# DavidHan008/SLAM-1

Hardware: AMD Instinct MI355X
Metric: frames/sec tracking+local-BA @1280x720 (higher is better)
Workload: dtype u8+f32+f64

## Files before the change

slam-1_amd/csrc/epnp.hpp:

```cpp
#pragma once

#include <hip/hip_runtime.h>
#include <cmath>
#include <cstddef>

namespace slam_epnp {

constexpr int EPNP_MAXN = 8;
constexpr int kEpnpWs = 4 * EPNP_MAXN + 48 + 60;

template <int n>
__device__ __forceinline__ void ep_jacobi(double* A, double* V) {
  #pragma unroll
  for (int i = 0; i < n; ++i)
    #pragma unroll
    for (int j = 0; j < n; ++j) V[i * n + j] = i == j ? 1.0 : 0.0;
  #pragma unroll 1
  for (int sweep = 0; sweep < 40; ++sweep) {
    double off = 0.0, dia = 0.0;
    #pragma unroll
    for (int i = 0; i < n; ++i) {
      dia += A[i * n + i] * A[i * n + i];
      #pragma unroll
      for (int j = i + 1; j < n; ++j) off += A[i * n + j] * A[i * n + j];
    }
    if (!(off > 1e-30 * dia)) break;
    constexpr int kUnroll = n <= 4 ? 4 : 1;
    #pragma unroll kUnroll
    for (int p = 0; p < n - 1; ++p)
      #pragma unroll kUnroll
      for (int q = p + 1; q < n; ++q) {
        const double apq = A[p * n + q];
        if (apq == 0.0) continue;
        const double app = A[p * n + p], aqq = A[q * n + q];
        const double th = (aqq - app) / (2.0 * apq);
        const double t = (th >= 0.0 ? 1.0 : -1.0) / (fabs(th) + sqrt(th * th + 1.0));
        const double c = 1.0 / sqrt(t * t + 1.0), s = t * c;
        #pragma unroll
        for (int k = 0; k < n; ++k) {
          const double akp = A[k * n + p], akq = A[k * n + q];
          A[k * n + p] = c * akp - s * akq;
          A[k * n + q] = s * akp + c * akq;
        }
        #pragma unroll
        for (int k = 0; k < n; ++k) {
          const double apk = A[p * n + k], aqk = A[q * n + k];
          A[p * n + k] = c * apk - s * aqk;
          A[q * n + k] = s * apk + c * aqk;
        }
        #pragma unroll
        for (int k = 0; k < n; ++k) {
          const double vkp = V[k * n + p], vkq = V[k * n + q];
          V[k * n + p] = c * vkp - s * vkq;
          V[k * n + q] = s * vkp + c * vkq;
        }
      }
  }
}

template <int k>
__device__ __forceinline__ int ep_lsq6(const double* A, const double* b, double* x) {
  double N[5][5], r[5];
  #pragma unroll
  for (int i = 0; i < k; ++i) {
    #pragma unroll
    for (int j = 0; j <= i; ++j) {
      double s = 0.0;
      #pragma unroll
      for (int m = 0; m < 6; ++m) s += A[m * k + i] * A[m * k + j];
      N[i][j] = s;
    }
    double s = 0.0;
    #pragma unroll
    for (int m = 0; m < 6; ++m) s += A[m * k + i] * b[m];
    r[i] = s;
  }
  #pragma unroll
  for (int j = 0; j < k; ++j) {
    double s = N[j][j];
    #pragma unroll
    for (int p = 0; p < j; ++p) s -= N[j][p] * N[j][p];
    if (!(s > 0.0)) return 0;
    N[j][j] = sqrt(s);
    #pragma unroll
    for (int i = j + 1; i < k; ++i) {
      double t = N[i][j];
      #pragma unroll
      for (int p = 0; p < j; ++p) t -= N[i][p] * N[j][p];
      N[i][j] = t / N[j][j];
    }
  }
  double y[5];
  #pragma unroll
  for (int i = 0; i < k; ++i) {
    double t = r[i];
    #pragma unroll
    for (int p = 0; p < i; ++p) t -= N[i][p] * y[p];
    y[i] = t / N[i][i];
  }
  #pragma unroll
  for (int i = k - 1; i >= 0; --i) {
    double t = y[i];
    #pragma unroll
    for (int p = i + 1; p < k; ++p) t -= N[p][i] * x[p];
    x[i] = t / N[i][i];
  }
  return 1;
}

// ... 72 lines not shown
  double c0[3] = {0, 0, 0}, w0[3] = {0, 0, 0};
  #pragma unroll
  for (int i = 0; i < n; ++i)
    #pragma unroll
    for (int d = 0; d < 3; ++d) {
      c0[d] += pc[i][d];
      w0[d] += pw[3 * i + d];
    }
  #pragma unroll
  for (int d = 0; d < 3; ++d) {
    c0[d] /= n;
    w0[d] /= n;
  }
  double S[3][3] = {{0, 0, 0}, {0, 0, 0}, {0, 0, 0}};
  #pragma unroll
  for (int i = 0; i < n; ++i)
    #pragma unroll
    for (int a = 0; a < 3; ++a)
      #pragma unroll
      for (int b = 0; b < 3; ++b) S[a][b] += (pw[3 * i + a] - w0[a]) * (pc[i][b] - c0[b]);
  double N[16] = {S[0][0] + S[1][1] + S[2][2], S[1][2] - S[2][1], S[2][0] - S[0][2], S[0][1] - S[1][0],
                  S[1][2] - S[2][1], S[0][0] - S[1][1] - S[2][2], S[0][1] + S[1][0], S[2][0] + S[0][2],
                  S[2][0] - S[0][2], S[0][1] + S[1][0], -S[0][0] + S[1][1] - S[2][2], S[1][2] + S[2][1],
                  S[0][1] - S[1][0], S[2][0] + S[0][2], S[1][2] + S[2][1], -S[0][0] - S[1][1] + S[2][2]};
  double V[16];
  ep_jacobi<4>(N, V);
  int bi = 0;
  #pragma unroll
  for (int i = 1; i < 4; ++i)
    if (N[i * 4 + i] > N[bi * 4 + bi]) bi = i;
  double q0 = V[0 * 4 + bi], q1 = V[1 * 4 + bi], q2 = V[2 * 4 + bi], q3 = V[3 * 4 + bi];
  if (q0 < 0.0) {
    q0 = -q0; q1 = -q1; q2 = -q2; q3 = -q3;
  }
  R[0] = q0 * q0 + q1 * q1 - q2 * q2 - q3 * q3;
  R[1] = 2.0 * (q1 * q2 - q0 * q3);
  R[2] = 2.0 * (q1 * q3 + q0 * q2);
  R[3] = 2.0 * (q1 * q2 + q0 * q3);
  R[4] = q0 * q0 - q1 * q1 + q2 * q2 - q3 * q3;
  R[5] = 2.0 * (q2 * q3 - q0 * q1);
  R[6] = 2.0 * (q1 * q3 - q0 * q2);
  R[7] = 2.0 * (q2 * q3 + q0 * q1);
  R[8] = q0 * q0 - q1 * q1 - q2 * q2 + q3 * q3;
  #pragma unroll
  for (int d = 0; d < 3; ++d) t[d] = c0[d] - (R[3 * d] * w0[0] + R[3 * d + 1] * w0[1] + R[3 * d + 2] * w0[2]);
  double err = 0.0;
  #pragma unroll
  for (int i = 0; i < n; ++i) {
    const double* X = pw + 3 * i;
    const double Xc = R[0] * X[0] + R[1] * X[1] + R[2] * X[2] + t[0];
    const double Yc = R[3] * X[0] + R[4] * X[1] + R[5] * X[2] + t[1];
    const double Zc = R[6] * X[0] + R[7] * X[1] + R[8] * X[2] + t[2];
    const double du = cx + fx * Xc / Zc - uv[2 * i], dv = cy + fy * Yc / Zc - uv[2 * i + 1];
    err += sqrt(du * du + dv * dv);
  }
  return err / n;
}

__device__ inline void ep_rvec(const double R[9], double r[3]) {
  const double tr = R[0] + R[4] + R[8];
  double q0, q1, q2, q3;
  if (tr > 0.0) {
    const double s = 2.0 * sqrt(tr + 1.0);
    q0 = 0.25 * s; q1 = (R[7] - R[5]) / s; q2 = (R[2] - R[6]) / s; q3 = (R[3] - R[1]) / s;
  } else if (R[0] > R[4] && R[0] > R[8]) {
    const double s = 2.0 * sqrt(1.0 + R[0] - R[4] - R[8]);
    q0 = (R[7] - R[5]) / s; q1 = 0.25 * s; q2 = (R[1] + R[3]) / s; q3 = (R[2] + R[6]) / s;
  } else if (R[4] > R[8]) {
    const double s = 2.0 * sqrt(1.0 + R[4] - R[0] - R[8]);
    q0 = (R[2] - R[6]) / s; q1 = (R[1] + R[3]) / s; q2 = 0.25 * s; q3 = (R[5] + R[7]) / s;
  } else {
    const double s = 2.0 * sqrt(1.0 + R[8] - R[0] - R[4]);
    q0 = (R[3] - R[1]) / s; q1 = (R[2] + R[6]) / s; q2 = (R[5] + R[7]) / s; q3 = 0.25 * s;
  }
  if (q0 < 0.0) {
    q0 = -q0; q1 = -q1; q2 = -q2; q3 = -q3;
  }
  const double vn = sqrt(q1 * q1 + q2 * q2 + q3 * q3);
  const double th = 2.0 * atan2(vn, q0);
  const double k = vn > 0.0 ? th / vn : 2.0;
  r[0] = q1 * k; r[1] = q2 * k; r[2] = q3 * k;
}

constexpr int kJld = 13;
struct EpGroup {
  double A[144], V[144];
  double alph[4 * EPNP_MAXN];
  double cw[4][3];
  double offdia[2];
  double B[2][12 * kJld];
  double cs[12];
  double part[24];
  double pad[3];
  int o12[4];
  int flag;
};
static_assert(sizeof(EpGroup) % 256 == 128, "EpGroup stride must be 128 mod 256 bytes");

struct EpBeta {
  double flag;
  double pw[3 * 5], uv[2 * 5];
  double alph[4 * 5];
  double cw[4][3];
  double v[4][12];
  double L[60], rho[6];
  double res[3][8];
};
constexpr int kEpRec = 1 + 15 + 10 + 20 + 12 + 48;
static_assert(offsetof(EpBeta, L) == kEpRec * sizeof(double), "EpBeta starts with the record");
static_assert(sizeof(EpBeta) % 64 == 32, "EpBeta stride must be 4 mod 8 doubles");

template <int n>
__device__ __forceinline__ int ep_bary(const double* pw, EpGroup& G) {
  double cw[4][3] = {{0, 0, 0}};
  for (int i = 0; i < n; ++i)
    for (int d = 0; d < 3; ++d) cw[0][d] += pw[3 * i + d];
  for (int d = 0; d < 3; ++d) cw[0][d] /= n;
  double A3[9] = {0, 0, 0, 0, 0, 0, 0, 0, 0}, V3[9];
  for (int i = 0; i < n; ++i)
    for (int a = 0; a < 3; ++a)
      for (int b = 0; b < 3; ++b) A3[3 * a + b] += (pw[3 * i + a] - cw[0][a]) * (pw[3 * i + b] - cw[0][b]);
  ep_jacobi<3>(A3, V3);
  int ord[3] = {0, 1, 2};
  for (int i = 0; i < 3; ++i)
    for (int j = i + 1; j < 3; ++j)
      if (A3[4 * ord[j]] > A3[4 * ord[i]]) {
        const int tmp = ord[i]; ord[i] = ord[j]; ord[j] = tmp;
      }
  for (int k = 0; k < 3; ++k) {
    const double sc = sqrt(fmax(A3[4 * ord[k]], 0.0) / n);
    for (int d = 0; d < 3; ++d) cw[k + 1][d] = cw[0][d] + sc * V3[3 * d + ord[k]];
  }
  for (int k = 0; k < 4; ++k)
    for (int d = 0; d < 3; ++d) G.cw[k][d] = cw[k][d];
  double C[3][3];
  for (int d = 0; d < 3; ++d)
    for (int k = 0; k < 3; ++k) C[d][k] = cw[k + 1][d] - cw[0][d];
  const double c00 = C[1][1] * C[2][2] - C[1][2] * C[2][1];
  const double c01 = C[0][2] * C[2][1] - C[0][1] * C[2][2];
  const double c02 = C[0][1] * C[1][2] - C[0][2] * C[1][1];
  const double c10 = C[1][2] * C[2][0] - C[1][0] * C[2][2];
  const double c11 = C[0][0] * C[2][2] - C[0][2] * C[2][0];
  const double c12 = C[0][2] * C[1][0] - C[0][0] * C[1][2];
  const double c20 = C[1][0] * C[2][1] - C[1][1] * C[2][0];
  const double c21 = C[0][1] * C[2][0] - C[0][0] * C[2][1];
  const double c22 = C[0][0] * C[1][1] - C[0][1] * C[1][0];
  const double det = C[0][0] * c00 + C[0][1] * c10 + C[0][2] * c20;
  if (!(fabs(det) > 0.0)) return 0;
  const double id = 1.0 / det;
  for (int i = 0; i < n; ++i) {
    const double x = pw[3 * i] - cw[0][0], y = pw[3 * i + 1] - cw[0][1], z = pw[3 * i + 2] - cw[0][2];
    const double a1 = (c00 * x + c01 * y + c02 * z) * id;
    const double a2 = (c10 * x + c11 * y + c12 * z) * id;
    const double a3 = (c20 * x + c21 * y + c22 * z) * id;
    G.alph[4 * i] = 1.0 - a1 - a2 - a3;
    G.alph[4 * i + 1] = a1;
    G.alph[4 * i + 2] = a2;
    G.alph[4 * i + 3] = a3;
  }
  return 1;
}

template <int n>
__device__ __forceinline__ void ep_mtm_row(int r, const double* uv, double fx, double fy, double cx,
                                           double cy, EpGroup& G) {
  double acc[12];
#pragma unroll
  for (int c = 0; c < 12; ++c) acc[c] = 0.0;
  const int jr = r / 3, dr = r - 3 * jr;
  for (int i = 0; i < n; ++i) {
    double m1[12], m2[12];
#pragma unroll
    for (int j = 0; j < 4; ++j) {
      const double a = G.alph[4 * i + j];
      m1[3 * j] = a * fx; m1[3 * j + 1] = 0.0; m1[3 * j + 2] = a * (cx - uv[2 * i]);
      m2[3 * j] = 0.0; m2[3 * j + 1] = a * fy; m2[3 * j + 2] = a * (cy - uv[2 * i + 1]);
    }
    const double ar = G.alph[4 * i + jr];
    const double m1r = dr == 0 ? ar * fx : dr == 1 ? 0.0 : ar * (cx - uv[2 * i]);
    const double m2r = dr == 0 ? 0.0 : dr == 1 ? ar * fy : ar * (cy - uv[2 * i + 1]);
#pragma unroll
    for (int c = 0; c < 12; ++c) acc[c] += m1r * m1[c] + m2r * m2[c];
  }
#pragma unroll
  for (int c = 0; c < 12; ++c) G.A[12 * r + c] = acc[c];
}

__device__ __forceinline__ void ep_pairs12(int r, int pp[6], int qq[6]) {
  int a[12];
  a[0] = 0;
#pragma unroll
  for (int i = 1; i < 12; ++i) a[i] = 1 + (i - 1 + r) % 11;
#pragma unroll
  for (int i = 0; i < 6; ++i) {
    const int x = a[i], y = a[11 - i];
    pp[i] = x < y ? x : y;
    qq[i] = x < y ? y : x;
  }
}

__device__ __forceinline__ void ep_rot_cs(double app, double aqq, double apq, double& c, double& s) {
  const bool z = apq == 0.0;
  const double th = (aqq - app) / (2.0 * (z ? 1.0 : apq));
  const double t = (th >= 0.0 ? 1.0 : -1.0) / (fabs(th) + sqrt(th * th + 1.0));
  const double cc = 1.0 / sqrt(t * t + 1.0);
  c = z ? 1.0 : cc;
  s = z ? 0.0 : t * cc;
}

template <int r>
__device__ __forceinline__ void ep_jacobi_round(EpGroup& G, int k, int kr, bool act, int cur,
                                                double (&vr)[12]) {
  constexpr int n = 12, ld = kJld;
  const double* A0 = G.B[cur];
  double* A1 = G.B[cur ^ 1];
  int pp[6], qq[6];
  ep_pairs12(r, pp, qq);
  if (k < 6) {
    const int x = k == 0 ? 0 : 1 + (k - 1 + r) % 11, y = 1 + (10 - k + r) % 11;
    const int p = x < y ? x : y, q = x < y ? y : x;
    double c, s;
    ep_rot_cs(A0[p * ld + p], A0[q * ld + q], A0[p * ld + q], c, s);
    G.cs[2 * k] = c;
    G.cs[2 * k + 1] = s;
  }
  const int pos = kr == 0 ? 0 : (kr + 10 - r % 11) % 11 + 1;
  const int ppos = 11 - pos;
  const int partner = ppos == 0 ? 0 : 1 + (ppos - 1 + r) % 11;
  const int pi = pos < ppos ? pos : ppos;
  const bool isp = kr < partner;
  double row[n], prow[n];
#pragma unroll
  for (int j = 0; j < n; ++j) {
    row[j] = A0[kr * ld + j];
    prow[j] = A0[partner * ld + j];
  }
  __syncthreads();
  double c[6], s[6];
#pragma unroll
  for (int i = 0; i < 6; ++i) {
    c[i] = G.cs[2 * i];
    s[i] = G.cs[2 * i + 1];
  }
  double ck = c[0], sk = s[0];
#pragma unroll
  for (int i = 1; i < 6; ++i) {
    ck = pi == i ? c[i] : ck;
    sk = pi == i ? s[i] : sk;
  }
  double out[n];
#pragma unroll
  for (int j = 0; j < n; ++j) out[j] = row[j];
#pragma unroll
  for (int i = 0; i < 6; ++i) {
    const int P = pp[i], Q = qq[i];
    const double akp = row[P], akq = row[Q];
    row[P] = c[i] * akp - s[i] * akq;
    row[Q] = s[i] * akp + c[i] * akq;
    const double bkp = prow[P], bkq = prow[Q];
    prow[P] = c[i] * bkp - s[i] * bkq;
    prow[Q] = s[i] * bkp + c[i] * bkq;
    const double vkp = vr[P], vkq = vr[Q];
    const double wp = c[i] * vkp - s[i] * vkq, wq = s[i] * vkp + c[i] * vkq;
    vr[P] = act ? wp : vkp;
    vr[Q] = act ? wq : vkq;
  }
#pragma unroll
  for (int j = 0; j < n; ++j) asm volatile("" : "+v"(vr[j]));
#pragma unroll
  for (int j = 0; j < n; ++j) {
    const double nv = isp ? ck * row[j] - sk * prow[j] : sk * prow[j] + ck * row[j];
    out[j] = act ? nv : out[j];
  }
  if (k < n) {
#pragma unroll
    for (int j = 0; j < n; ++j) A1[k * ld + j] = out[j];
  }
  __syncthreads();
}

__device__ __forceinline__ void ep_jacobi12_group(EpGroup& G, int k, bool live) {
  constexpr int n = 12, ld = kJld;
  const bool own = k < n;
  const int kr = own ? k : 0;
  double vr[n];
#pragma unroll
  for (int j = 0; j < n; ++j) vr[j] = kr == j ? 1.0 : 0.0;
  if (own) {
#pragma unroll
    for (int j = 0; j < n; ++j) G.B[0][k * ld + j] = G.A[k * n + j];
  }
  if (k == 0) G.flag = live ? 1 : 0;
  __syncthreads();
  int cur = 0;
  for (int sweep = 0; sweep < 40; ++sweep) {
    if (own) {
      const double* Ar = G.B[cur] + k * ld;
      double o = 0.0;
#pragma unroll
      for (int j = 1; j < n; ++j)
        if (j > k) o += Ar[j] * Ar[j];
      G.part[k] = Ar[k] * Ar[k];
      G.part[n + k] = o;
    }
    __syncthreads();
    if (k == 0 && G.flag) {
      double off = 0.0, dia = 0.0;
      for (int i = 0; i < n; ++i) {
        dia += G.part[i];
        off += G.part[n + i];
      }
      if (!(off > 1e-24 * dia)) G.flag = 0;
    }
    __syncthreads();
    const bool act = own && G.flag != 0;
    if (__ballot(G.flag != 0) == 0ull) break;
#ifdef SLAM_PNPH_TRACE
    if (threadIdx.x == 0) G.offdia[1] = sweep + 1;
#endif
    ep_jacobi_round<0>(G, k, kr, act, cur, vr);
    ep_jacobi_round<1>(G, k, kr, act, cur ^ 1, vr);
    ep_jacobi_round<2>(G, k, kr, act, cur, vr);
    ep_jacobi_round<3>(G, k, kr, act, cur ^ 1, vr);
    ep_jacobi_round<4>(G, k, kr, act, cur, vr);
    ep_jacobi_round<5>(G, k, kr, act, cur ^ 1, vr);
    ep_jacobi_round<6>(G, k, kr, act, cur, vr);
    ep_jacobi_round<7>(G, k, kr, act, cur ^ 1, vr);
    ep_jacobi_round<8>(G, k, kr, act, cur, vr);
    ep_jacobi_round<9>(G, k, kr, act, cur ^ 1, vr);
    ep_jacobi_round<10>(G, k, kr, act, cur, vr);
    cur ^= 1;
  }
  if (own) {
#pragma unroll
    for (int j = 0; j < n; ++j) {
      G.A[k * n + j] = G.B[cur][k * ld + j];
      G.V[k * n + j] = vr[j];
    }
  }
  __syncthreads();
}

__device__ __forceinline__ void ep_order(EpGroup& G) {
  int o12[12];
  for (int i = 0; i < 12; ++i) o12[i] = i;
  for (int i = 0; i < 4; ++i)
    for (int j = i + 1; j < 12; ++j)
      if (G.A[13 * o12[j]] < G.A[13 * o12[i]]) {
        const int tmp = o12[i]; o12[i] = o12[j]; o12[j] = tmp;
      }
  for (int k = 0; k < 4; ++k) G.o12[k] = o12[k];
}

__device__ __forceinline__ void ep_lrho(EpBeta& G) {
  const int pa[6] = {0, 0, 0, 1, 1, 2}, pb[6] = {1, 2, 3, 2, 3, 3};
  for (int j = 0; j < 6; ++j) {
    double dv[4][3];
    for (int k = 0; k < 4; ++k)
      for (int d = 0; d < 3; ++d) dv[k][d] = G.v[k][3 * pa[j] + d] - G.v[k][3 * pb[j] + d];
#define EP_DOT(a, b) (dv[a][0] * dv[b][0] + dv[a][1] * dv[b][1] + dv[a][2] * dv[b][2])
    G.L[10 * j + 0] = EP_DOT(0, 0);
    G.L[10 * j + 1] = 2.0 * EP_DOT(0, 1);
    G.L[10 * j + 2] = EP_DOT(1, 1);
    G.L[10 * j + 3] = 2.0 * EP_DOT(0, 2);
    G.L[10 * j + 4] = 2.0 * EP_DOT(1, 2);
    G.L[10 * j + 5] = EP_DOT(2, 2);
    G.L[10 * j + 6] = 2.0 * EP_DOT(0, 3);
    G.L[10 * j + 7] = 2.0 * EP_DOT(1, 3);
    G.L[10 * j + 8] = 2.0 * EP_DOT(2, 3);
    G.L[10 * j + 9] = EP_DOT(3, 3);
#undef EP_DOT
    double s = 0.0;
    for (int d = 0; d < 3; ++d) {
      const double e = G.cw[pa[j]][d] - G.cw[pb[j]][d];
      s += e * e;
    }
    G.rho[j] = s;
  }
}

template <int n>
__device__ __forceinline__ void ep_approx(int approx, const double* pw, const double* uv, double fx,
                                          double fy, double cx, double cy, EpBeta& G) {
  double* res = G.res[approx];
  res[7] = 0.0;
  const int k = approx == 0 ? 4 : approx == 1 ? 3 : 5;
  double As[30], xb[5], rho[6];
#pragma unroll
  for (int j = 0; j < 6; ++j) rho[j] = G.rho[j];
#pragma unroll
  for (int j = 0; j < 6; ++j)
#pragma unroll
    for (int c = 0; c < 5; ++c) {
      const int col = c < 2 ? c : approx == 0 ? (c == 2 ? 3 : 6) : c;
      As[j * 5 + c] = c < k ? G.L[10 * j + col] : 0.0;
    }
  if (!ep_lsq6_live(As, rho, k, xb)) return;
  double be[4] = {0, 0, 0, 0};
  if (approx == 0) {
    if (xb[0] < 0.0) {
      be[0] = sqrt(-xb[0]);
      be[1] = -xb[1] / be[0]; be[2] = -xb[2] / be[0]; be[3] = -xb[3] / be[0];
    } else {
      be[0] = sqrt(xb[0]);
      be[1] = xb[1] / be[0]; be[2] = xb[2] / be[0]; be[3] = xb[3] / be[0];
    }
  } else {
    if (xb[0] < 0.0) {
      be[0] = sqrt(-xb[0]);
      be[1] = xb[2] < 0.0 ? sqrt(-xb[2]) : 0.0;
    } else {
      be[0] = sqrt(xb[0]);
      be[1] = xb[2] > 0.0 ? sqrt(xb[2]) : 0.0;
    }
    if (xb[1] < 0.0) be[0] = -be[0];
    if (approx == 2) be[2] = xb[3] / be[0];
  }
#pragma unroll 1
  for (int it = 0; it < 5; ++it) {
    double Ag[24], bg[6], dx[4];
    int lo = 0;
    asm volatile("" : "+v"(lo));
    for (int j = 0; j < 6; ++j) {
      const double* l = G.L + 10 * j + lo;
      Ag[4 * j + 0] = 2.0 * l[0] * be[0] + l[1] * be[1] + l[3] * be[2] + l[6] * be[3];
      Ag[4 * j + 1] = l[1] * be[0] + 2.0 * l[2] * be[1] + l[4] * be[2] + l[7] * be[3];
      Ag[4 * j + 2] = l[3] * be[0] + l[4] * be[1] + 2.0 * l[5] * be[2] + l[8] * be[3];
      Ag[4 * j + 3] = l[6] * be[0] + l[7] * be[1] + l[8] * be[2] + 2.0 * l[9] * be[3];
      bg[j] = rho[j] - (l[0] * be[0] * be[0] + l[1] * be[0] * be[1] + l[2] * be[1] * be[1] +
                        l[3] * be[0] * be[2] + l[4] * be[1] * be[2] + l[5] * be[2] * be[2] +
                        l[6] * be[0] * be[3] + l[7] * be[1] * be[3] + l[8] * be[2] * be[3] +
// ... 36 lines not shown
```

slam-1_amd/csrc/geometry.hip:

```cpp
#include "common.hpp"
#include "epnp.hpp"
#include "dlt.hpp"
#include "pose_math.hpp"

#include <climits>

#include <cmath>

namespace {

constexpr int kBS = 256;

__global__ __launch_bounds__(kBS) void k_gather(const float* __restrict__ kpq, int kq_cap,
                                                const float* __restrict__ kpt, int kt_cap,
                                                const uint8_t* __restrict__ dq_in,
                                                const uint8_t* __restrict__ dt_in,
                                                const int2* __restrict__ pairs,
                                                const int32_t* __restrict__ count, int p_cap,
                                                double* __restrict__ ptq, double* __restrict__ ptt,
                                                uint8_t* __restrict__ dq, uint8_t* __restrict__ dt) {
  const int b = blockIdx.y;
  const int n = min(max(count[b], 0), p_cap);
  const int k = blockIdx.x * kBS + threadIdx.x;
  if (k >= n) return;
// ... 72 lines not shown
  uint64_t z = s;
  z = (z ^ (z >> 30)) * 0xBF58476D1CE4E5B9ull;
  z = (z ^ (z >> 27)) * 0x94D049BB133111EBull;
  return z ^ (z >> 31);
}

constexpr int kMinSample = 5;
constexpr int kPnPWG = 256;
constexpr int kMaxHyp = 256;
constexpr int kRc = 4;

constexpr int kLmT = 29;
constexpr int kLmGroup = 304;
static_assert(kLmGroup >= 2 * kMinSample * kLmT && (2 * kLmGroup) % 64 == 32, "lm_group LDS layout");
__device__ void lm_group(const double* Q, const double* q, int n, const Cam& K, int iters,
                         double p[6], int k, double (*t)[kLmT], double* sums) {
  double lam = 1e-3;
  double R[9];
  rodrigues(p, R);
  for (int it = 0; it < iters; ++it) {
    if (k < n) {
      double r[2], J[2][6];
      pnp_residual<true>(p, R, Q + 3 * k, q + 2 * k, K, r, J);
#pragma unroll
      for (int a = 0; a < 2; ++a) {
        double* o = t[2 * k + a];
        int m = 0;
#pragma unroll
        for (int u = 0; u < 6; ++u) {
#pragma unroll
          for (int v = 0; v <= u; ++v) o[m++] = J[a][u] * J[a][v];
          o[21 + u] = J[a][u] * r[a];
        }
        o[27] = r[a] * r[a];
      }
    }
    __syncthreads();
#pragma unroll
    for (int e = 0; e < 2; ++e) {
      const int j = k + 16 * e;
      if (j < 28) {
        double acc = 0.0;
        for (int sa = 0; sa < 2 * n; ++sa) acc += t[sa][j];
        sums[j] = acc;
      }
    }
    __syncthreads();
    double H[21], g[6];
#pragma unroll
    for (int i = 0; i < 21; ++i) H[i] = sums[i];
#pragma unroll
    for (int i = 0; i < 6; ++i) g[i] = sums[21 + i];
    const double cost = sums[27];
    double d[6], pn[6];
    const bool ok = solve6(H, g, lam, d);
    if (!ok) {
      lam = fmin(lam * 10.0, 1e12);
      __syncthreads();
      continue;
    }
    for (int i = 0; i < 6; ++i) pn[i] = p[i] + d[i];
    double Rn[9];
    rodrigues(pn, Rn);
    __syncthreads();
    if (k < n) {
      double r[2], J[2][6];
      pnp_residual<false>(pn, Rn, Q + 3 * k, q + 2 * k, K, r, J);
      sums[k] = r[0] * r[0] + r[1] * r[1];
    }
    __syncthreads();
    double cn = 0.0;
    for (int s2 = 0; s2 < n; ++s2) cn += sums[s2];
    __syncthreads();
    if (cn < cost) {
      for (int i = 0; i < 6; ++i) p[i] = pn[i];
      for (int i = 0; i < 9; ++i) R[i] = Rn[i];
      lam = fmax(lam * 0.1, 1e-12);
    } else {
      lam = fmin(lam * 10.0, 1e12);
    }
  }
}

constexpr int kHypGroups = 4;
constexpr int kBetaGroups = 16;
constexpr int kEpRec = slam_epnp::kEpRec;
#ifdef SLAM_PNPH_TRACE
__device__ unsigned long long g_pnph[16];
#define PNPH_T(i) do { if (threadIdx.x == 0 && blockIdx.x == 3 && blockIdx.y == 5) g_pnph[i] = __builtin_amdgcn_s_memtime(); } while (0)
#else
#define PNPH_T(i) (void)0
#endif
__device__ void pnp_sample(uint64_t seed, int item, int h, int L, const double* Q, const double* q,
                           double* pw, double* uv, int* sidx) {
  uint64_t s = seed ^ ((uint64_t)item * 0xD1B54A32D192ED03ull) ^
               ((uint64_t)h * 0x8CB92BA72F3D8DD7ull);
  int idx[kMinSample];
  for (int kk = 0; kk < kMinSample; ++kk) {
    int v;
    bool dup;
    do {
      v = (int)((splitmix64(s) >> 32) % (uint64_t)L);
      dup = false;
      for (int j = 0; j < kk; ++j) dup |= idx[j] == v;
    } while (dup);
    idx[kk] = v;
    sidx[kk] = v;
    for (int d = 0; d < 3; ++d) pw[3 * kk + d] = Q[3 * v + d];
    for (int d = 0; d < 2; ++d) uv[2 * kk + d] = q[2 * v + d];
  }
}

__global__ __launch_bounds__(64) void k_pnp_hyp_eig(const double* __restrict__ Qall,
                                                    const double* __restrict__ qall,
                                                    const int32_t* __restrict__ count, int cap,
                                                    const double* __restrict__ Kp, uint64_t seed,
                                                    int item0, int n_hyp,
                                                    double* __restrict__ scr) {
#ifdef SLAM_PNP_PRIO
  __builtin_amdgcn_s_setprio(SLAM_PNP_PRIO);
#endif
  __shared__ slam_epnp::EpGroup grp[kHypGroups];
  __shared__ double spw[kHypGroups][3 * kMinSample], suv[kHypGroups][2 * kMinSample];
  __shared__ int sidx[kHypGroups][kMinSample];
  const int b = blockIdx.x, t = threadIdx.x;
  const int g = t >> 4, k = t & 15;
  const int h = blockIdx.y * kHypGroups + g;
  const int L = min(max(count[b], 0), cap);
  if (L < kMinSample) return;
  const bool live = h < n_hyp;
  const double* Q = Qall + (size_t)b * cap * 3;
  const double* q = qall + (size_t)b * cap * 2;
  const Cam K{Kp[0], Kp[4], Kp[2], Kp[5]};
  slam_epnp::EpGroup& G = grp[g];
  PNPH_T(0);
  if (k == 0 && live) {
    pnp_sample(seed, item0 + b, h, L, Q, q, spw[g], suv[g], sidx[g]);
    G.flag = slam_epnp::ep_bary<kMinSample>(spw[g], G);
  }
  __syncthreads();
  PNPH_T(1);
  bool ok = live && G.flag != 0;
  if (ok && k < 12) slam_epnp::ep_mtm_row<kMinSample>(k, suv[g], K.fx, K.fy, K.cx, K.cy, G);
  __syncthreads();
  PNPH_T(2);
  slam_epnp::ep_jacobi12_group(G, k, ok);
  PNPH_T(3);
#ifdef SLAM_PNPH_TRACE
  if (threadIdx.x == 0 && blockIdx.x == 3 && blockIdx.y == 5) g_pnph[7] = (unsigned long long)G.offdia[1];
#endif
  if (ok && k == 0) slam_epnp::ep_order(G);
  __syncthreads();
  if (live) {
    double* rec = scr + ((size_t)b * n_hyp + h) * kEpRec;
    if (k == 0) rec[0] = ok ? 1.0 : 0.0;
    if (ok) {
      if (k < 3 * kMinSample) rec[1 + k] = spw[g][k];
      if (k < 2 * kMinSample) rec[16 + k] = suv[g][k];
      for (int i = k; i < 4 * kMinSample; i += 16) rec[26 + i] = G.alph[i];
      if (k < 12) {
        rec[46 + k] = G.cw[k / 3][k % 3];
        for (int kk = 0; kk < 4; ++kk) rec[58 + 12 * kk + k] = G.V[12 * k + G.o12[kk]];
      }
    }
  }
  PNPH_T(4);
}

__global__ __launch_bounds__(64) void k_pnp_hyp_beta(const int32_t* __restrict__ count, int cap,
                                                     const double* __restrict__ Kp, int n_hyp,
                                                     const double* __restrict__ scr,
                                                     double* __restrict__ ws) {
#ifdef SLAM_PNP_PRIO
  __builtin_amdgcn_s_setprio(SLAM_PNP_PRIO);
#endif
  __shared__ slam_epnp::EpBeta grp[kBetaGroups];
  const int b = blockIdx.x, t = threadIdx.x;
  const int g = t >> 2, k = t & 3;
  const int h0 = blockIdx.y * kBetaGroups, h = h0 + g;
  const int L = min(max(count[b], 0), cap);
  if (L < kMinSample) return;
  const bool live = h < n_hyp;
  const Cam K{Kp[0], Kp[4], Kp[2], Kp[5]};
  slam_epnp::EpBeta& G = grp[g];
  PNPH_T(8);
  {
    const double* src = scr + ((size_t)b * n_hyp + h0) * kEpRec;
    const int nrec = min(kBetaGroups, n_hyp - h0) * kEpRec;
    for (int i = t; i < nrec; i += 64) {
      const int gi = i / kEpRec;
      reinterpret_cast<double*>(&grp[gi])[i - gi * kEpRec] = src[i];
    }
  }
  __syncthreads();
  PNPH_T(9);
  const bool ok = live && G.flag != 0.0;
  if (ok && k == 0) slam_epnp::ep_lrho(G);
  __syncthreads();
  PNPH_T(10);
  if (ok && k < 3) slam_epnp::ep_approx<kMinSample>(k, G.pw, G.uv, K.fx, K.fy, K.cx, K.cy, G);
  __syncthreads();
  PNPH_T(11);
  if (k == 0 && live) {
    double p[6] = {0, 0, 0, 0, 0, 0};
    if (!(ok && slam_epnp::ep_choose(G, p)))
      for (int i = 0; i < 6; ++i) p[i] = 0.0;
    double* o = ws + ((size_t)b * n_hyp + h) * 6;
    for (int i = 0; i < 6; ++i) o[i] = p[i];
  }
  PNPH_T(12);
}

__global__ __launch_bounds__(64) void k_pnp_hyp_lm(const double* __restrict__ Qall,
                                                   const double* __restrict__ qall,
                                                   const int32_t* __restrict__ count, int cap,
                                                   const double* __restrict__ Kp, uint64_t seed,
                                                   int item0, int n_hyp, int hyp_iters,
                                                   double* __restrict__ ws) {
#ifdef SLAM_PNP_PRIO
  __builtin_amdgcn_s_setprio(SLAM_PNP_PRIO);
#endif
  __shared__ double spw[kHypGroups][3 * kMinSample], suv[kHypGroups][2 * kMinSample];
  __shared__ int sidx[kHypGroups][kMinSample];
  __shared__ double lmt[kHypGroups * kLmGroup], lms[kHypGroups][28 + kMinSample];
  __shared__ double p0[kHypGroups][6];
  const int b = blockIdx.x, t = threadIdx.x;
  const int g = t >> 4, k = t & 15;
  const int h = blockIdx.y * kHypGroups + g;
  const int L = min(max(count[b], 0), cap);
  if (L < kMinSample) return;
  const bool live = h < n_hyp;
  const double* Q = Qall + (size_t)b * cap * 3;
  const double* q = qall + (size_t)b * cap * 2;
  const Cam K{Kp[0], Kp[4], Kp[2], Kp[5]};
  double* o = ws + ((size_t)b * n_hyp + (live ? h : 0)) * 6;
  if (k == 0) {
    if (live) pnp_sample(seed, item0 + b, h, L, Q, q, spw[g], suv[g], sidx[g]);
    else
      for (int i = 0; i < 3 * kMinSample; ++i) spw[g][i] = suv[g][i % (2 * kMinSample)] = 0.0;
  }
  if (k < 6) p0[g][k] = live ? o[k] : 0.0;
  __syncthreads();
  double p[6];
  for (int i = 0; i < 6; ++i) p[i] = p0[g][i];
  lm_group(spw[g], suv[g], kMinSample, K, hyp_iters, p, k,
// ... 563 lines not shown
  k_gather<<<grid, kBS, 0, slam::as_stream(stream)>>>(
      d_kpq, kq_cap, d_kpt, kt_cap, d_desq, d_dest, reinterpret_cast<const int2*>(d_pairs),
      d_count, p_cap, d_ptq, d_ptt, d_dq, d_dt);
  SLAM_LAUNCHED("k_gather");
  return SLAM_OK;
}

extern "C" int slam_gather_temporal(const double* d_X, const double* d_ptl, int xcap,
                                    const float* d_kp_next, int kcap, const int32_t* d_pairs,
                                    const int32_t* d_count, int pcap, int batch, double* d_Q1,
                                    double* d_q2, double* d_q1, void* stream) {
  SLAM_REQUIRE(batch >= 0 && pcap >= 0 && xcap >= 0 && kcap >= 0,
               "slam_gather_temporal: bad shape");
  if (batch == 0 || pcap == 0) return SLAM_OK;
  SLAM_REQUIRE(d_X && d_ptl && d_kp_next && d_pairs && d_count && d_Q1 && d_q2 && d_q1,
               "slam_gather_temporal: null pointer");
  dim3 grid((pcap + kBS - 1) / kBS, batch);
  k_gather_temporal<<<grid, kBS, 0, slam::as_stream(stream)>>>(
      d_X, d_ptl, xcap, d_kp_next, kcap, reinterpret_cast<const int2*>(d_pairs), d_count, pcap,
      d_Q1, d_q2, d_q1);
  SLAM_LAUNCHED("k_gather_temporal");
  return SLAM_OK;
}

extern "C" int slam_triangulate(const double* d_ptl, const double* d_ptr, const int32_t* d_count,
                                int cap, int batch, const double* d_Pl, const double* d_Pr,
                                int proj_stride, double* d_X, void* stream) {
  SLAM_REQUIRE(batch >= 0 && cap >= 0, "slam_triangulate: bad shape");
  SLAM_REQUIRE(proj_stride == 0 || proj_stride == 12, "slam_triangulate: proj_stride 0 or 12");
  if (batch == 0 || cap == 0) return SLAM_OK;
  SLAM_REQUIRE(d_ptl && d_ptr && d_count && d_Pl && d_Pr && d_X, "slam_triangulate: null pointer");
  dim3 grid((cap + kBS - 1) / kBS, batch);
  k_triangulate<<<grid, kBS, 0, slam::as_stream(stream)>>>(d_ptl, d_ptr, d_count, cap, d_Pl, d_Pr,
                                                           proj_stride, d_X);
  SLAM_LAUNCHED("k_triangulate");
  return SLAM_OK;
}

extern "C" long long slam_pnp_workspace_len(int batch, int n_hyp) {
  return (long long)batch * n_hyp * 6;
}

static int pnp_check_args(const double* d_Q, const double* d_q, const int32_t* d_count, int cap,
                          int batch, const double* d_K, int n_hyp, double reproj_thresh,
                          int hyp_iters, int refine_iters, const double* d_rvec,
                          const double* d_tvec, const int32_t* d_ninliers, const uint8_t* d_mask,
                          const double* d_ws, long long ws_len) {
  SLAM_REQUIRE(batch >= 0 && cap >= 0, "slam_pnp_ransac: bad shape");
  SLAM_REQUIRE(n_hyp >= 1 && n_hyp <= kMaxHyp, "slam_pnp_ransac: n_hyp in [1, %d]", kMaxHyp);
  SLAM_REQUIRE(hyp_iters >= 0 && refine_iters >= 0 && reproj_thresh > 0,
               "slam_pnp_ransac: bad iteration/threshold arguments");
  if (batch == 0) return SLAM_OK;
  SLAM_REQUIRE(d_Q && d_q && d_count && d_K && d_rvec && d_tvec && d_ninliers && d_mask && d_ws,
               "slam_pnp_ransac: null pointer");
  if (ws_len < slam_pnp_workspace_len(batch, n_hyp)) {
    slam::set_error("slam_pnp_ransac: workspace %lld < %lld doubles", ws_len,
                    slam_pnp_workspace_len(batch, n_hyp));
    return SLAM_ERR_WORKSPACE;
  }
  return SLAM_OK;
}

extern "C" long long slam_pnp_scratch_len(int batch, int n_hyp) {
  return (long long)(batch > 0 ? batch : 0) * (n_hyp > 0 ? n_hyp : 0) * kEpRec;
}

extern "C" int slam_pnp_ransac_ws(const double* d_Q, const double* d_q, const int32_t* d_count,
                                  int cap, int batch, const double* d_K, uint64_t seed, int item0,
                                  int n_hyp, double reproj_thresh, int hyp_iters, int refine_iters,
                                  double* d_rvec, double* d_tvec, int32_t* d_ninliers,
                                  uint8_t* d_mask, double* d_ws, long long ws_len,
                                  double* d_scratch, long long scratch_len, void* stream) {
  if (int rc = pnp_check_args(d_Q, d_q, d_count, cap, batch, d_K, n_hyp, reproj_thresh, hyp_iters,
                              refine_iters, d_rvec, d_tvec, d_ninliers, d_mask, d_ws, ws_len))
    return rc;
  if (batch == 0) return SLAM_OK;
  SLAM_REQUIRE(d_scratch != nullptr, "slam_pnp_ransac: null scratch");
  if (scratch_len < slam_pnp_scratch_len(batch, n_hyp)) {
    slam::set_error("slam_pnp_ransac: scratch %lld < %lld doubles", scratch_len,
                    slam_pnp_scratch_len(batch, n_hyp));
    return SLAM_ERR_WORKSPACE;
  }
  hipStream_t s = slam::as_stream(stream);
  const dim3 egrid(batch, (n_hyp + kHypGroups - 1) / kHypGroups);
  k_pnp_hyp_eig<<<egrid, 64, 0, s>>>(d_Q, d_q, d_count, cap, d_K, seed, item0, n_hyp, d_scratch);
  SLAM_LAUNCHED("k_pnp_hyp_eig");
  const dim3 bgrid(batch, (n_hyp + kBetaGroups - 1) / kBetaGroups);
  k_pnp_hyp_beta<<<bgrid, 64, 0, s>>>(d_count, cap, d_K, n_hyp, d_scratch, d_ws);
  SLAM_LAUNCHED("k_pnp_hyp_beta");
  k_pnp_hyp_lm<<<egrid, 64, 0, s>>>(d_Q, d_q, d_count, cap, d_K, seed, item0, n_hyp, hyp_iters,
                                    d_ws);
  SLAM_LAUNCHED("k_pnp_hyp_lm");
  k_pnp<<<batch, kPnPWG, 0, s>>>(d_Q, d_q, d_count, cap, d_K, seed, item0, n_hyp, reproj_thresh,
                                 hyp_iters, refine_iters, d_rvec, d_tvec, d_ninliers, d_mask,
                                 d_ws);
  SLAM_LAUNCHED("k_pnp");
  return SLAM_OK;
}

extern "C" int slam_pnp_ransac(const double* d_Q, const double* d_q, const int32_t* d_count,
                               int cap, int batch, const double* d_K, uint64_t seed, int item0,
                               int n_hyp, double reproj_thresh, int hyp_iters, int refine_iters,
                               double* d_rvec, double* d_tvec, int32_t* d_ninliers,
                               uint8_t* d_mask, double* d_ws, long long ws_len, void* stream) {
  if (int rc = pnp_check_args(d_Q, d_q, d_count, cap, batch, d_K, n_hyp, reproj_thresh, hyp_iters,
                              refine_iters, d_rvec, d_tvec, d_ninliers, d_mask, d_ws, ws_len))
    return rc;
  if (batch == 0) return SLAM_OK;
  hipStream_t s = slam::as_stream(stream);
  const long long n = slam_pnp_scratch_len(batch, n_hyp);
  double* scr = nullptr;
  SLAM_HIP(hipMallocAsync(reinterpret_cast<void**>(&scr), (size_t)n * sizeof(double), s));
  const int rc = slam_pnp_ransac_ws(d_Q, d_q, d_count, cap, batch, d_K, seed, item0, n_hyp,
                                    reproj_thresh, hyp_iters, refine_iters, d_rvec, d_tvec,
                                    d_ninliers, d_mask, d_ws, ws_len, scr, n, s);
  SLAM_HIP(hipFreeAsync(scr, s));
  return rc;
}

extern "C" int slam_vo_pose_workspace_bytes(int batch, int max_iter, size_t* bytes) {
  SLAM_REQUIRE(batch >= 0 && max_iter >= 1 && bytes, "slam_vo_pose_workspace_bytes: bad args");
  *bytes = (size_t)batch * max_iter * 7 * sizeof(double) + 256;
  return SLAM_OK;
}

extern "C" int slam_vo_estimate_pose(const double* d_q1, const double* d_q2, const double* d_Q1,
                                     const double* d_Q2, const int32_t* d_count, int cap,
                                     int batch, const double* d_P, uint64_t seed, int item0,
                                     int max_iter, int lm_iters, int early_stop, double* d_pose,
                                     int32_t* d_best, int32_t* d_ntried, double* d_err,
                                     void* d_ws, size_t ws_bytes, void* stream) {
  SLAM_REQUIRE(batch >= 0 && cap >= 0, "slam_vo_estimate_pose: bad shape");
  SLAM_REQUIRE(max_iter >= 1 && max_iter <= kVoWG, "slam_vo_estimate_pose: max_iter in [1, %d]",
               kVoWG);
  SLAM_REQUIRE(lm_iters >= 0 && early_stop >= 1, "slam_vo_estimate_pose: bad lm_iters/early_stop");
  if (batch == 0) return SLAM_OK;
  SLAM_REQUIRE(d_q1 && d_q2 && d_Q1 && d_Q2 && d_count && d_P && d_pose && d_best && d_ntried &&
                   d_err,
               "slam_vo_estimate_pose: null pointer");
  SLAM_REQUIRE(d_ws != nullptr, "slam_vo_estimate_pose: null workspace");
  size_t need = 0;
  if (int rc = slam_vo_pose_workspace_bytes(batch, max_iter, &need)) return rc;
  if (ws_bytes < need) {
    slam::set_error("slam_vo_estimate_pose: workspace %zu < %zu bytes", ws_bytes, need);
    return SLAM_ERR_WORKSPACE;
  }
  double* ws_pp = static_cast<double*>(d_ws);
  double* ws_err = ws_pp + (size_t)batch * max_iter * 6;
  hipStream_t s = slam::as_stream(stream);
  k_vo_hyp<<<batch, kVoWG, 0, s>>>(d_q1, d_q2, d_Q1, d_Q2, d_count, cap, d_P, seed, item0,
                                   max_iter, lm_iters, ws_pp);
  SLAM_LAUNCHED("k_vo_hyp");
  const size_t lds = sizeof(double) * (size_t)min(2 * cap, kNpChunk);
  k_vo_err<<<dim3(max_iter, batch), kErrWG, lds, s>>>(d_q1, d_q2, d_Q1, d_Q2, d_count, cap, d_P,
                                                      max_iter, ws_pp, ws_err);
  SLAM_LAUNCHED("k_vo_err");
  k_vo_select<<<(batch + 63) / 64, 64, 0, s>>>(d_count, cap, batch, max_iter, early_stop, ws_pp,
                                               ws_err, d_pose, d_best, d_ntried, d_err);
  SLAM_LAUNCHED("k_vo_select");
  return SLAM_OK;
}

extern "C" int slam_vo_residuals(const double* d_dof, const double* d_q1, const double* d_q2,
                                 const double* d_Q1, const double* d_Q2, const int32_t* d_count,
                                 int cap, int batch, const double* d_P, double* d_res,
                                 void* stream) {
  SLAM_REQUIRE(batch >= 0 && cap >= 0, "slam_vo_residuals: bad shape");
  if (batch == 0 || cap == 0) return SLAM_OK;
  SLAM_REQUIRE(d_dof && d_q1 && d_q2 && d_Q1 && d_Q2 && d_count && d_P && d_res,
               "slam_vo_residuals: null pointer");
  dim3 grid((4 * cap + kBS - 1) / kBS, batch);
  k_vo_residuals<<<grid, kBS, 0, slam::as_stream(stream)>>>(d_dof, d_q1, d_q2, d_Q1, d_Q2,
                                                           d_count, cap, d_P, d_res);
// ... 24 lines not shown
```

Measured before the change: 24700.

## Pack five EPnP hypotheses per wave with in-place interleaved Jacobi matrix

Result: faster. 24960, median of 6 (+1.1%).

```diff
diff --git a/slam-1_amd/csrc/epnp.hpp b/slam-1_amd/csrc/epnp.hpp
--- a/slam-1_amd/csrc/epnp.hpp
+++ b/slam-1_amd/csrc/epnp.hpp
@@ -9,12 +9,13 @@
 constexpr int EPNP_MAXN = 8;
 constexpr int kEpnpWs = 4 * EPNP_MAXN + 48 + 60;
 
-template <int n>
+template <int n, bool kWaveExit = false>
 __device__ __forceinline__ void ep_jacobi(double* A, double* V) {
   #pragma unroll
   for (int i = 0; i < n; ++i)
     #pragma unroll
     for (int j = 0; j < n; ++j) V[i * n + j] = i == j ? 1.0 : 0.0;
+  bool done = false;
   #pragma unroll 1
   for (int sweep = 0; sweep < 40; ++sweep) {
     double off = 0.0, dia = 0.0;
@@ -24,7 +25,13 @@
       #pragma unroll
       for (int j = i + 1; j < n; ++j) off += A[i * n + j] * A[i * n + j];
     }
-    if (!(off > 1e-30 * dia)) break;
+    if (kWaveExit) {
+      done = done || !(off > 1e-30 * dia);
+      if (__ballot(!done) == 0ull) break;
+      if (done) continue;
+    } else if (!(off > 1e-30 * dia)) {
+      break;
+    }
     constexpr int kUnroll = n <= 4 ? 4 : 1;
     #pragma unroll kUnroll
     for (int p = 0; p < n - 1; ++p)
@@ -263,20 +270,23 @@
   r[0] = q1 * k; r[1] = q2 * k; r[2] = q3 * k;
 }
 
-constexpr int kJld = 13;
+constexpr int kEigLanes = 12;
+constexpr int kEigGroups = 64 / kEigLanes;
 struct EpGroup {
-  double A[144], V[144];
   double alph[4 * EPNP_MAXN];
   double cw[4][3];
   double offdia[2];
-  double B[2][12 * kJld];
   double cs[12];
   double part[24];
-  double pad[3];
+  double pad[23];
   int o12[4];
   int flag;
 };
-static_assert(sizeof(EpGroup) % 256 == 128, "EpGroup stride must be 128 mod 256 bytes");
+static_assert(sizeof(EpGroup) % 256 == 96, "EpGroup stride must be 12 mod 32 doubles");
+constexpr int kJl = 12 * kEigGroups;
+struct EpJacobi {
+  double B[12 * kJl];
+};
 
 struct EpBeta {
   double flag;
@@ -301,7 +311,7 @@
   for (int i = 0; i < n; ++i)
     for (int a = 0; a < 3; ++a)
       for (int b = 0; b < 3; ++b) A3[3 * a + b] += (pw[3 * i + a] - cw[0][a]) * (pw[3 * i + b] - cw[0][b]);
-  ep_jacobi<3>(A3, V3);
+  ep_jacobi<3, true>(A3, V3);
   int ord[3] = {0, 1, 2};
   for (int i = 0; i < 3; ++i)
     for (int j = i + 1; j < 3; ++j)
@@ -344,7 +354,7 @@
 
 template <int n>
 __device__ __forceinline__ void ep_mtm_row(int r, const double* uv, double fx, double fy, double cx,
-                                           double cy, EpGroup& G) {
+                                           double cy, const EpGroup& G, double* J) {
   double acc[12];
 #pragma unroll
   for (int c = 0; c < 12; ++c) acc[c] = 0.0;
@@ -364,7 +374,7 @@
     for (int c = 0; c < 12; ++c) acc[c] += m1r * m1[c] + m2r * m2[c];
   }
 #pragma unroll
-  for (int c = 0; c < 12; ++c) G.A[12 * r + c] = acc[c];
+  for (int c = 0; c < 12; ++c) J[c * kJl + r] = acc[c];
 }
 
 __device__ __forceinline__ void ep_pairs12(int r, int pp[6], int qq[6]) {
@@ -389,19 +399,18 @@
   s = z ? 0.0 : t * cc;
 }
 
+constexpr int kJacAhead = 1;
 template <int r>
-__device__ __forceinline__ void ep_jacobi_round(EpGroup& G, int k, int kr, bool act, int cur,
+__device__ __forceinline__ void ep_jacobi_round(EpGroup& G, double* J, int k, int kr, bool act,
                                                 double (&vr)[12]) {
-  constexpr int n = 12, ld = kJld;
-  const double* A0 = G.B[cur];
-  double* A1 = G.B[cur ^ 1];
+  constexpr int n = 12, ld = kJl;
   int pp[6], qq[6];
   ep_pairs12(r, pp, qq);
   if (k < 6) {
     const int x = k == 0 ? 0 : 1 + (k - 1 + r) % 11, y = 1 + (10 - k + r) % 11;
     const int p = x < y ? x : y, q = x < y ? y : x;
     double c, s;
-    ep_rot_cs(A0[p * ld + p], A0[q * ld + q], A0[p * ld + q], c, s);
+    ep_rot_cs(J[p * ld + p], J[q * ld + q], J[q * ld + p], c, s);
     G.cs[2 * k] = c;
     G.cs[2 * k + 1] = s;
   }
@@ -410,78 +419,61 @@
   const int partner = ppos == 0 ? 0 : 1 + (ppos - 1 + r) % 11;
   const int pi = pos < ppos ? pos : ppos;
   const bool isp = kr < partner;
-  double row[n], prow[n];
-#pragma unroll
-  for (int j = 0; j < n; ++j) {
-    row[j] = A0[kr * ld + j];
-    prow[j] = A0[partner * ld + j];
+  double akp[6], akq[6], bkp[6], bkq[6];
+#pragma unroll
+  for (int i = 0; i < kJacAhead; ++i) {
+    akp[i] = J[pp[i] * ld + kr];
+    akq[i] = J[qq[i] * ld + kr];
+    bkp[i] = J[pp[i] * ld + partner];
+    bkq[i] = J[qq[i] * ld + partner];
   }
   __syncthreads();
-  double c[6], s[6];
-#pragma unroll
-  for (int i = 0; i < 6; ++i) {
-    c[i] = G.cs[2 * i];
-    s[i] = G.cs[2 * i + 1];
-  }
-  double ck = c[0], sk = s[0];
-#pragma unroll
-  for (int i = 1; i < 6; ++i) {
-    ck = pi == i ? c[i] : ck;
-    sk = pi == i ? s[i] : sk;
-  }
-  double out[n];
-#pragma unroll
-  for (int j = 0; j < n; ++j) out[j] = row[j];
+  const double ck = G.cs[2 * pi], sk = G.cs[2 * pi + 1];
 #pragma unroll
   for (int i = 0; i < 6; ++i) {
     const int P = pp[i], Q = qq[i];
-    const double akp = row[P], akq = row[Q];
-    row[P] = c[i] * akp - s[i] * akq;
-    row[Q] = s[i] * akp + c[i] * akq;
-    const double bkp = prow[P], bkq = prow[Q];
-    prow[P] = c[i] * bkp - s[i] * bkq;
-    prow[Q] = s[i] * bkp + c[i] * bkq;
+    if (i + kJacAhead < 6) {
+      const int j = i + kJacAhead;
+      akp[j] = J[pp[j] * ld + kr];
+      akq[j] = J[qq[j] * ld + kr];
+      bkp[j] = J[pp[j] * ld + partner];
+      bkq[j] = J[qq[j] * ld + partner];
+    }
+    const double c = G.cs[2 * i], s = G.cs[2 * i + 1];
+    const double rp = c * akp[i] - s * akq[i], rq = s * akp[i] + c * akq[i];
+    const double tp = c * bkp[i] - s * bkq[i], tq = s * bkp[i] + c * bkq[i];
     const double vkp = vr[P], vkq = vr[Q];
-    const double wp = c[i] * vkp - s[i] * vkq, wq = s[i] * vkp + c[i] * vkq;
+    const double wp = c * vkp - s * vkq, wq = s * vkp + c * vkq;
     vr[P] = act ? wp : vkp;
     vr[Q] = act ? wq : vkq;
-  }
-#pragma unroll
-  for (int j = 0; j < n; ++j) asm volatile("" : "+v"(vr[j]));
-#pragma unroll
-  for (int j = 0; j < n; ++j) {
-    const double nv = isp ? ck * row[j] - sk * prow[j] : sk * prow[j] + ck * row[j];
-    out[j] = act ? nv : out[j];
-  }
-  if (k < n) {
-#pragma unroll
-    for (int j = 0; j < n; ++j) A1[k * ld + j] = out[j];
+    asm volatile("" : "+v"(vr[P]), "+v"(vr[Q]));
+    const double np = isp ? ck * rp - sk * tp : sk * tp + ck * rp;
+    const double nq = isp ? ck * rq - sk * tq : sk * tq + ck * rq;
+    if (k < n) {
+      J[P * ld + k] = act ? np : akp[i];
+      J[Q * ld + k] = act ? nq : akq[i];
+    }
   }
   __syncthreads();
 }
 
-__device__ __forceinline__ void ep_jacobi12_group(EpGroup& G, int k, bool live) {
-  constexpr int n = 12, ld = kJld;
+__device__ __forceinline__ void ep_jacobi12_group(EpGroup& G, double* J, int k, bool live,
+                                                  double (&vr)[12]) {
+  constexpr int n = 12, ld = kJl;
   const bool own = k < n;
   const int kr = own ? k : 0;
-  double vr[n];
 #pragma unroll
   for (int j = 0; j < n; ++j) vr[j] = kr == j ? 1.0 : 0.0;
-  if (own) {
-#pragma unroll
-    for (int j = 0; j < n; ++j) G.B[0][k * ld + j] = G.A[k * n + j];
-  }
   if (k == 0) G.flag = live ? 1 : 0;
   __syncthreads();
-  int cur = 0;
   for (int sweep = 0; sweep < 40; ++sweep) {
     if (own) {
-      const double* Ar = G.B[cur] + k * ld;
+      const double* Ar = J + k;
       double o = 0.0;
 #pragma unroll
       for (int j = 1; j < n; ++j)
-        if (j > k) o += Ar[j] * Ar[j];
-      G.part[k] = Ar[k] * Ar[k];
+        if (j > k) o += Ar[j * ld] * Ar[j * ld];
+      G.part[k] = Ar[k * ld] * Ar[k * ld];
       G.part[n + k] = o;
     }
     __syncthreads();
@@ -499,35 +491,28 @@
 #ifdef SLAM_PNPH_TRACE
     if (threadIdx.x == 0) G.offdia[1] = sweep + 1;
 #endif
-    ep_jacobi_round<0>(G, k, kr, act, cur, vr);
-    ep_jacobi_round<1>(G, k, kr, act, cur ^ 1, vr);
-    ep_jacobi_round<2>(G, k, kr, act, cur, vr);
-    ep_jacobi_round<3>(G, k, kr, act, cur ^ 1, vr);
-    ep_jacobi_round<4>(G, k, kr, act, cur, vr);
-    ep_jacobi_round<5>(G, k, kr, act, cur ^ 1, vr);
-    ep_jacobi_round<6>(G, k, kr, act, cur, vr);
-    ep_jacobi_round<7>(G, k, kr, act, cur ^ 1, vr);
-    ep_jacobi_round<8>(G, k, kr, act, cur, vr);
-    ep_jacobi_round<9>(G, k, kr, act, cur ^ 1, vr);
-    ep_jacobi_round<10>(G, k, kr, act, cur, vr);
-    cur ^= 1;
-  }
-  if (own) {
-#pragma unroll
-    for (int j = 0; j < n; ++j) {
-      G.A[k * n + j] = G.B[cur][k * ld + j];
-      G.V[k * n + j] = vr[j];
-    }
-  }
-  __syncthreads();
-}
-
-__device__ __forceinline__ void ep_order(EpGroup& G) {
+    int ko = k, ro = kr;
+    asm volatile("" : "+v"(ko), "+v"(ro));
+    ep_jacobi_round<0>(G, J, ko, ro, act, vr);
+    ep_jacobi_round<1>(G, J, ko, ro, act, vr);
+    ep_jacobi_round<2>(G, J, ko, ro, act, vr);
+    ep_jacobi_round<3>(G, J, ko, ro, act, vr);
+    ep_jacobi_round<4>(G, J, ko, ro, act, vr);
+    ep_jacobi_round<5>(G, J, ko, ro, act, vr);
+    ep_jacobi_round<6>(G, J, ko, ro, act, vr);
+    ep_jacobi_round<7>(G, J, ko, ro, act, vr);
+    ep_jacobi_round<8>(G, J, ko, ro, act, vr);
+    ep_jacobi_round<9>(G, J, ko, ro, act, vr);
+    ep_jacobi_round<10>(G, J, ko, ro, act, vr);
+  }
+}
+
+__device__ __forceinline__ void ep_order(EpGroup& G, const double* J) {
   int o12[12];
   for (int i = 0; i < 12; ++i) o12[i] = i;
   for (int i = 0; i < 4; ++i)
     for (int j = i + 1; j < 12; ++j)
-      if (G.A[13 * o12[j]] < G.A[13 * o12[i]]) {
+      if (J[(kJl + 1) * o12[j]] < J[(kJl + 1) * o12[i]]) {
         const int tmp = o12[i]; o12[i] = o12[j]; o12[j] = tmp;
       }
   for (int k = 0; k < 4; ++k) G.o12[k] = o12[k];
diff --git a/slam-1_amd/csrc/geometry.hip b/slam-1_amd/csrc/geometry.hip
--- a/slam-1_amd/csrc/geometry.hip
+++ b/slam-1_amd/csrc/geometry.hip
@@ -178,6 +178,8 @@
   }
 }
 
+constexpr int kEigGroups = slam_epnp::kEigGroups;
+constexpr int kEigLanes = slam_epnp::kEigLanes;
 constexpr int kHypGroups = 4;
 constexpr int kBetaGroups = 16;
 constexpr int kEpRec = slam_epnp::kEpRec;
@@ -216,15 +218,18 @@
 #ifdef SLAM_PNP_PRIO
   __builtin_amdgcn_s_setprio(SLAM_PNP_PRIO);
 #endif
-  __shared__ slam_epnp::EpGroup grp[kHypGroups];
-  __shared__ double spw[kHypGroups][3 * kMinSample], suv[kHypGroups][2 * kMinSample];
-  __shared__ int sidx[kHypGroups][kMinSample];
+  __shared__ slam_epnp::EpGroup grp[kEigGroups];
+  __shared__ slam_epnp::EpJacobi jac;
+  __shared__ double spw[kEigGroups][3 * kMinSample], suv[kEigGroups][2 * kMinSample];
+  __shared__ int sidx[kEigGroups][kMinSample];
   const int b = blockIdx.x, t = threadIdx.x;
-  const int g = t >> 4, k = t & 15;
-  const int h = blockIdx.y * kHypGroups + g;
+  const bool idle = t >= kEigGroups * kEigLanes;
+  const int g = idle ? kEigGroups - 1 : t / kEigLanes;
+  const int k = idle ? kEigLanes : t - g * kEigLanes;
+  const int h = blockIdx.y * kEigGroups + g;
   const int L = min(max(count[b], 0), cap);
   if (L < kMinSample) return;
-  const bool live = h < n_hyp;
+  const bool live = !idle && h < n_hyp;
   const double* Q = Qall + (size_t)b * cap * 3;
   const double* q = qall + (size_t)b * cap * 2;
   const Cam K{Kp[0], Kp[4], Kp[2], Kp[5]};
@@ -237,26 +242,34 @@
   __syncthreads();
   PNPH_T(1);
   bool ok = live && G.flag != 0;
-  if (ok && k < 12) slam_epnp::ep_mtm_row<kMinSample>(k, suv[g], K.fx, K.fy, K.cx, K.cy, G);
+  double* J = jac.B + 12 * g;
+  if (ok && k < 12) slam_epnp::ep_mtm_row<kMinSample>(k, suv[g], K.fx, K.fy, K.cx, K.cy, G, J);
   __syncthreads();
   PNPH_T(2);
-  slam_epnp::ep_jacobi12_group(G, k, ok);
+  double vr[12];
+  slam_epnp::ep_jacobi12_group(G, J, k, ok, vr);
   PNPH_T(3);
 #ifdef SLAM_PNPH_TRACE
   if (threadIdx.x == 0 && blockIdx.x == 3 && blockIdx.y == 5) g_pnph[7] = (unsigned long long)G.offdia[1];
 #endif
-  if (ok && k == 0) slam_epnp::ep_order(G);
+  if (ok && k == 0) slam_epnp::ep_order(G, J);
   __syncthreads();
   if (live) {
     double* rec = scr + ((size_t)b * n_hyp + h) * kEpRec;
     if (k == 0) rec[0] = ok ? 1.0 : 0.0;
     if (ok) {
-      if (k < 3 * kMinSample) rec[1 + k] = spw[g][k];
-      if (k < 2 * kMinSample) rec[16 + k] = suv[g][k];
-      for (int i = k; i < 4 * kMinSample; i += 16) rec[26 + i] = G.alph[i];
+      for (int i = k; i < 3 * kMinSample; i += kEigLanes) rec[1 + i] = spw[g][i];
+      for (int i = k; i < 2 * kMinSample; i += kEigLanes) rec[16 + i] = suv[g][i];
+      for (int i = k; i < 4 * kMinSample; i += kEigLanes) rec[26 + i] = G.alph[i];
       if (k < 12) {
         rec[46 + k] = G.cw[k / 3][k % 3];
-        for (int kk = 0; kk < 4; ++kk) rec[58 + 12 * kk + k] = G.V[12 * k + G.o12[kk]];
+        for (int kk = 0; kk < 4; ++kk) {
+          const int o = G.o12[kk];
+          double v = vr[0];
+#pragma unroll
+          for (int j = 1; j < 12; ++j) v = o == j ? vr[j] : v;
+          rec[58 + 12 * kk + k] = v;
+        }
       }
     }
   }
@@ -986,13 +999,14 @@
     return SLAM_ERR_WORKSPACE;
   }
   hipStream_t s = slam::as_stream(stream);
-  const dim3 egrid(batch, (n_hyp + kHypGroups - 1) / kHypGroups);
+  const dim3 egrid(batch, (n_hyp + kEigGroups - 1) / kEigGroups);
   k_pnp_hyp_eig<<<egrid, 64, 0, s>>>(d_Q, d_q, d_count, cap, d_K, seed, item0, n_hyp, d_scratch);
   SLAM_LAUNCHED("k_pnp_hyp_eig");
   const dim3 bgrid(batch, (n_hyp + kBetaGroups - 1) / kBetaGroups);
   k_pnp_hyp_beta<<<bgrid, 64, 0, s>>>(d_count, cap, d_K, n_hyp, d_scratch, d_ws);
   SLAM_LAUNCHED("k_pnp_hyp_beta");
-  k_pnp_hyp_lm<<<egrid, 64, 0, s>>>(d_Q, d_q, d_count, cap, d_K, seed, item0, n_hyp, hyp_iters,
+  const dim3 lgrid(batch, (n_hyp + kHypGroups - 1) / kHypGroups);
+  k_pnp_hyp_lm<<<lgrid, 64, 0, s>>>(d_Q, d_q, d_count, cap, d_K, seed, item0, n_hyp, hyp_iters,
                                     d_ws);
   SLAM_LAUNCHED("k_pnp_hyp_lm");
   k_pnp<<<batch, kPnPWG, 0, s>>>(d_Q, d_q, d_count, cap, d_K, seed, item0, n_hyp, reproj_thresh,
```
